# iacopo97/Multimodal-SAM-Adapter

Hardware: AMD Instinct MI355X
Metric: images/sec encoder fwd @1024x1024 RGB+LiDAR ViT-L (higher is better)
Workload: dtype split-operand MFMA: fp16 hi + e5m2 cross terms (h8c / h8 planes, ViT / interaction / up-conv GEMMs) fp16 hi/lo pairs x3 (TwinConvNeXt: f3 planes) and bf16 hi/lo x3 (neck, head); attention blocks with the rel-pos terms fused: every contraction on one fp16 MFMA (q, k, v, P rounded to fp16) in the bloc

## Files before the change

include/mmsa.h:

```cpp
#ifndef MMSA_H
#define MMSA_H
#include <stddef.h>
#include <stdint.h>
#ifdef __cplusplus
extern "C" {
#endif

#ifdef MMSA_BUILDING_LIBRARY
typedef hipStream_t mmsa_stream_t;
#else
typedef void* mmsa_stream_t;
#endif

#include "mmsa_version.h"
int mmsa_version(void);
const char* mmsa_last_error(void);

int mmsa_debug_poison_lds(unsigned pattern, mmsa_stream_t stream);
int mmsa_event_create(void** ev);
int mmsa_event_record(void* ev, mmsa_stream_t stream);
int mmsa_event_elapsed_ms(void* start, void* stop, float* ms);
int mmsa_event_destroy(void* ev);

enum { MMSA_ACT_NONE = 0, MMSA_ACT_GELU = 1, MMSA_ACT_RELU = 2, MMSA_ACT_RELU6 = 3, MMSA_ACT_HSWISH = 4, MMSA_ACT_SIGMOID = 5 };

enum { MMSA_DT_F32 = 0, MMSA_DT_F16 = 1, MMSA_DT_F64 = 2 };

enum { MMSA_FMT_B3 = 0, MMSA_FMT_H8 = 1, MMSA_FMT_H8C = 2, MMSA_FMT_F3 = 3, MMSA_FMT_W8 = 4  };

int mmsa_ms_deform_attn_forward(const void* value, const int64_t* spatial_shapes, const int64_t* level_start_index,
                                const void* sampling_loc, const void* attn_weight, void* out, int batch,
                                int spatial_size, int num_heads, int channels, int num_levels, int num_query,
                                int num_point, int im2col_step, int dtype, mmsa_stream_t stream);

int mmsa_ms_deform_attn_backward(const void* value, const int64_t* spatial_shapes, const int64_t* level_start_index,
                                 const void* sampling_loc, const void* attn_weight, const void* grad_output,
                                 void* grad_value, void* grad_sampling_loc, void* grad_attn_weight, int batch,
                                 int spatial_size, int num_heads, int channels, int num_levels, int num_query,
                                 int num_point, int im2col_step, int dtype, mmsa_stream_t stream);

int mmsa_msda_fused(const float* value, const int64_t* spatial_shapes, const int64_t* level_start_index,
                    const float* raw, long ldraw, const float* ref_points, float* out, long ldo,
                    uint16_t* out_planes, long ldop , int out_fmt , int batch,
                    int spatial_size, int num_heads, int channels, int num_levels, int num_query, int num_point,
                    float* clamp_max , mmsa_stream_t stream);

int mmsa_msda_fused_planes(const uint16_t* value_planes, long ldvp, int lo_bytes, const int64_t* spatial_shapes, const int64_t* level_start_index,
                           const float* raw, long ldraw, const float* ref_points, float* out, long ldo,
                           uint16_t* out_planes, long ldop, int out_fmt, int batch,
                           int spatial_size, int num_heads, int channels, int num_levels, int num_query, int num_point,
                           float* clamp_max, mmsa_stream_t stream);

int mmsa_rowstats_finalize(const float* rowstats, int rows, int strips, int D, float eps, float* mean_rstd, mmsa_stream_t stream);

int mmsa_zero_bytes(void* p, size_t bytes, mmsa_stream_t stream);
int mmsa_gemm_split3(const float* A, const uint16_t* Ap, long lda, long strideA,
                     const uint16_t* Wp, long strideW,
                     const float* bias, long strideBias, const float* colscale, const float* resid, long ldr,
                     long strideR, int resid_mod, float beta, float* C, long ldc, long strideC,
                     uint16_t* Cp, long ldcp, long strideCp, int M, int N, int K,
                     int batch, int act, float alpha, int out_mode, int ps_H, int ps_W, int ps_C, int fmt, int cp_fmt,
                     int max_grid, float* rowstats_out, const float* rownorm_mean_rstd, const float* rownorm_colsum, int flavour,
                     float* clamp_max , mmsa_stream_t stream);

int mmsa_convnext_mlp_fused(const uint16_t* Ap, long lda, long strideA, const uint16_t* W1p, long strideW1, const uint16_t* W2p,
                            long strideW2, const float* b1, const float* b2, const float* gamma, float* x, long ldx, long strideX,
                            int M, int C, int batch, int max_grid, int fmt,
                            float* clamp_max , mmsa_stream_t stream);

int mmsa_split_planes(const float* src, long ld, int rows, int cols, int cols_pad, uint16_t* planes, int kind,
                      float* clamp_max , mmsa_stream_t stream);

int mmsa_attention(const float* qkv, long ldq, const float* qkv_bias, const float* rp, float* out, long ldo, int B,
                   int H, int W, int heads, int head_dim, int window_size, float scale, mmsa_stream_t stream);
int mmsa_attention_planes(const uint16_t* qkv_planes, long ldq, const uint16_t* bias_planes, const float* rp,
                          uint16_t* out_planes, long ldo, int B, int H, int W, int heads, int head_dim,
                          int window_size, float scale, int out_fmt ,
                          int v_fmt ,
                          float* max_abs_logit , mmsa_stream_t stream);

int mmsa_relpos_bias(const float* qkv, long ldq, const float* Rh, const float* Rw, float* rp, int B, int H, int W,
                     int heads, int head_dim, int window_size, mmsa_stream_t stream);
int mmsa_relpos_bias_planes(const uint16_t* qkv_planes, long ldq, const float* Rh, const float* Rw,
                            float* rp, int B, int H, int W, int heads, int head_dim, int window_size, mmsa_stream_t stream);

int mmsa_layernorm_rows(const float* x, long ldx, const float* w, const float* b, float eps, float* y, long ldy,
                        float* y2, long ldy2, uint16_t* y_planes, long ldp ,
                        int rows, int C, int map_mode, int map_H, int map_W, int group_rows, long w_gstride, long y_gcol,
                        int y_wrap, int plane_fmt , float* clamp_max ,
                        mmsa_stream_t stream);

int mmsa_colstats(const float* x, long ldx, long strideB, const float* wrow, int B, int HW, int C, double* out,
                  int out_is_zero , mmsa_stream_t stream);

int mmsa_ffrm_finalize(const double* stats, int B, int HW, int C, float mean_w, float mean_b, const float* Wc,
                       const float* gn_w, const float* gn_b, float* mean_o, float* rstd_o, float* mult_o,
                       float* scratch , mmsa_stream_t stream);
int mmsa_lnhw_apply(const float* x, long ldx, const float* mean, const float* rstd, const float* mult, const float* w,
                    const float* bias, float* y, long ldy, int B, int HW, int C, mmsa_stream_t stream);

int mmsa_dwconv_nhwc(const float* x, long ldx, long xstrideB, const float* w, const float* bias, float* y, long ldy,
                     long ystrideB, uint16_t* y_planes, long ldp, long pstrideB , int planes_fmt ,
                     int B, int H, int W, int C, int k, int act,
                     int imgs_per_group ,
                     float* rowstats ,
                     float* clamp_max , mmsa_stream_t stream);
int mmsa_gconv_nhwc(const float* x, long ldx, const float* w, const float* bias, float* y, long ldy, int B, int H,
                    int W, int G, int cin_g, int cout_g, int k, int act, mmsa_stream_t stream);
int mmsa_gfe_qkv_conv(const float* x, long ldx, const float* w, float* y, long ldy, int B, int H, int W, int G, int cin_g, int cout_g,
                      int* covered, mmsa_stream_t stream);
int mmsa_dwpair_gate(const float* x, long ldx, const float* w, float* y, long ldy, uint16_t* y_planes, long ldp, int B, int H,
                     int W, int C, mmsa_stream_t stream);
int mmsa_im2col_nchw(const float* x, int B, int Ctot, int c0, int Cin, int H, int W, int p, float* out, int Kpad,
                     mmsa_stream_t stream);

long mmsa_gram_tn_scratch_bytes(int B, int P, int c);
int mmsa_gram_tn(const float* X, long ldx, const float* Y, long ldy, long strideB, double* G , int B, int P, int c,
                 int nblk, void* scratch, long scratch_bytes, mmsa_stream_t stream);
int mmsa_chanattn_build(const double* G, const double* sq, long sq_strideB, const double* sk, long sk_strideB,
                        const float* temp, const float* Wp, uint16_t* planes , int B, int c, int cpad,
                        int heads, mmsa_stream_t stream);
int mmsa_gffm_build(const double* E, uint16_t* x_planes, uint16_t* y_planes , int B, int c,
                    int cpad, mmsa_stream_t stream);
int mmsa_gelu_gate(const float* x, long ldx, float* y, long ldy, long rows, int C, mmsa_stream_t stream);
int mmsa_pool_hw(const float* z, long ldz, float* out, long ldo, int B, int H, int W, int C, mmsa_stream_t stream);
int mmsa_ca_apply(const float* z, long ldz, const float* att, long lda, float* out, long ldo,
                  uint16_t* out_planes, long ldp , int B, int H, int W, int C, mmsa_stream_t stream);

int mmsa_tail_fuse(const float* cmap, long ldc, long cstrideB, const float* xtok, long ldx, const float* bn_scale,
                   const float* bn_shift, float* out, uint16_t* out_planes , long ldp,
                   int B, int Hc, int Wc, int Hx, int Wx, int C, mmsa_stream_t stream);

int mmsa_global_attention_planes(const uint16_t* qkv_planes, long ldq, const uint16_t* bias_planes, const uint16_t* relpos_planes,
                                 uint16_t* out_planes, long ldo, int B, int H, int W, int heads, int head_dim, float scale,
                                 int out_fmt , int v_fmt ,
                                 float* max_abs_logit , mmsa_stream_t stream);

int mmsa_window_attention_planes(const uint16_t* qkv_planes, long ldq, const uint16_t* bias_planes,
                                 const uint16_t* relpos_planes, const uint16_t* selector, uint16_t* out_planes, long ldo, int B, int H, int W,
                                 int heads, int head_dim, int window_size, float scale, int out_fmt ,
                                 int v_fmt , float* max_abs_logit , mmsa_stream_t stream);

int mmsa_nchw_to_planes(const float* src, long strideB, uint16_t* planes, long ldp, int B, int C, long HW,
                        mmsa_stream_t stream);
int mmsa_head_fuse(const float* z0, const float* z1, int H1, int W1, const float* z2, int H2, int W2, const float* z3,
                   int H3, int W3, long ld, const float* bn_scale, const float* bn_shift, uint16_t* planes, long ldp,
                   float* out32, long ldo, int B, int H, int W, int C, int act, mmsa_stream_t stream);
int mmsa_tokens_to_nchw(const float* src, long ld, float* dst, int B, long HW, int C, mmsa_stream_t stream);

int mmsa_bilinear_accum_nchw(const float* src, long src_strideB, int B, int C, int hs, int ws, float* dst, int Hd, int Wd, int y0, int x0,
                             int hc, int wc, float* count, int accumulate, mmsa_stream_t stream);
int mmsa_div_count_nchw(float* x, const float* count, int B, int C, long HW, mmsa_stream_t stream);
int mmsa_argmax_nchw(const float* x, unsigned char* out, int B, int C, long HW, mmsa_stream_t stream);
int mmsa_crop_batch_nchw(const float* src, int B, int C, int H, int W, const int* windows, int n, float* dst, int hc, int wc,
                         mmsa_stream_t stream);
int mmsa_slide_argmax(const float* logits, int n, int C, int hs, int ws, const int* windows, unsigned char* out, int B, int H, int W,
                      int hc, int wc, int* uncovered, mmsa_stream_t stream);
int mmsa_slide_argmax_resized(const float* logits, int n, int C, int hs, int ws, const int* windows, unsigned char* out, int B, int H, int W,
                              int hc, int wc, int Hd, int Wd, int Hcut, int Wcut, int* uncovered, mmsa_stream_t stream);

int mmsa_softmax_flip_accum_nchw(const float* logits, float* acc, int B, int C, int H, int W, int flip, int accumulate, int finish_div, mmsa_stream_t stream);
int mmsa_aug_argmax(const float* const* logits, const int* views, int A, int C, const int* windows, const int* windows_host, int total,
                    unsigned char* out, int B, int Ho, int Wo, int* uncovered, mmsa_stream_t stream);

enum { MMSA_PRE_U8 = 0, MMSA_PRE_F32 = 1 };
int mmsa_preprocess_nhwc(const void* src0, int dtype0, const void* src1, int dtype1, int B, int Hs, int Ws, const float* mean,
                         const float* sinv, const int* div255, const int* swap, const float* pad_val, float* dst, int H, int W,
                         mmsa_stream_t stream);
int mmsa_preprocess_crops(const void* src0, int dtype0, const void* src1, int dtype1, int B, int Hs, int Ws, const float* mean,
                          const float* sinv, const int* div255, const int* swap, const float* pad_val, int H, int W, const int* windows,
                          int n, float* dst, int hc, int wc, mmsa_stream_t stream);
int mmsa_preprocess_resize_nhwc(const void* src0, int dtype0, const void* src1, int dtype1, int B, int Hs, int Ws, const float* mean,
                                const float* sinv, const int* div255, const int* swap, const float* pad_val, float* dst, int H, int W,
                                int Hr, int Wr, const int* xofs, const void* xcoef, const int* yofs, const void* ycoef, int fixed_point,
                                mmsa_stream_t stream);
int mmsa_preprocess_resize_crops(const void* src0, int dtype0, const void* src1, int dtype1, int B, int Hs, int Ws, const float* mean,
                                 const float* sinv, const int* div255, const int* swap, const float* pad_val, int H, int W, const int* windows,
                                 int n, float* dst, int hc, int wc, int Hr, int Wr, const int* xofs, const void* xcoef, const int* yofs,
                                 const void* ycoef, int fixed_point, mmsa_stream_t stream);

int mmsa_eval_confusion_u8(const unsigned char* pred, const unsigned char* label, int B, int H, int W, int Hl, int Wl, const unsigned char* lut,
                           int C, const int* ymap, const int* xmap, const int* slots, int n_slots, int64_t* counts, mmsa_stream_t stream);
int mmsa_slide_argmax_eval(const float* logits, int n, int C, int hs, int ws, const int* windows, unsigned char* out, int B, int H, int W,
                           int hc, int wc, int* uncovered, const unsigned char* label, int Hl, int Wl, const unsigned char* lut, const int* ymap,
                           const int* xmap, const int* slots, int n_slots, int64_t* counts, mmsa_stream_t stream);

int mmsa_render_u8(const unsigned char* pred, long pred_image_stride, long pred_row_stride, int B, int h, int w, const unsigned* palette, int npal,
                   int palette_reverse, const unsigned char* src, int Hs, int Ws, int src_reverse, double opacity, double one_minus_opacity,
                   unsigned char* out, mmsa_stream_t stream);
int mmsa_render_denorm_f32(const unsigned char* pred, long pred_image_stride, long pred_row_stride, int B, int h, int w, const unsigned* palette, int npal,
                           int palette_reverse, const float* src, int Cs, int Hs, int Ws, const float* mean, const float* std, int to_rgb, int mul255,
                           double opacity, double one_minus_opacity, unsigned char* out, mmsa_stream_t stream);

#ifdef __cplusplus
}
#endif
#endif
```

include/mmsa_version.h:

```cpp
#ifndef MMSA_VERSION_H
#define MMSA_VERSION_H
#define MMSA_ABI_VERSION 110
#endif
```

multimodal-sam-adapter_amd/csrc/head.hip:

```cpp
#include "common.h"

template <bool VEC>
__global__ __launch_bounds__(256) void nchw_to_planes_kernel(const float* __restrict__ src, long strideB, int C, long HW,
                                                             uint16_t* __restrict__ planes, long ldp) {
  __shared__ float tile[32][257];
  const int b = blockIdx.z;
  const long pix0 = (long)blockIdx.x * 256;
  const int c0 = blockIdx.y * 32;
  const int lane = threadIdx.x & 63, wv = threadIdx.x >> 6;
  const float* sb = src + (long)b * strideB;
  if (VEC) {
    float4 v[8];
#pragma unroll
    for (int j = 0; j < 8; ++j) {
      const int c = c0 + wv * 8 + j;
      const long pix = pix0 + 4 * lane;
      v[j] = (c < C && pix < HW) ? *reinterpret_cast<const float4*>(sb + (long)c * HW + pix) : make_float4(0.f, 0.f, 0.f, 0.f);
    }
#pragma unroll
    for (int j = 0; j < 8; ++j) {
      float* t = &tile[wv * 8 + j][4 * lane];
      t[0] = v[j].x; t[1] = v[j].y; t[2] = v[j].z; t[3] = v[j].w;
    }
  } else {
#pragma unroll
    for (int j = 0; j < 8; ++j) {
      const int cl = wv * 8 + j;
      const int c = c0 + cl;
#pragma unroll
      for (int k = 0; k < 4; ++k) {
        const long pix = pix0 + lane + 64 * k;
        tile[cl][lane + 64 * k] = (c < C && pix < HW) ? sb[(long)c * HW + pix] : 0.f;
      }
    }
  }
  __syncthreads();
  const int q = threadIdx.x & 3;
  const int pl = threadIdx.x >> 2;
#pragma unroll
  for (int k = 0; k < 4; ++k) {
    const int p = pl + 64 * k;
    const long pix = pix0 + p;
    if (pix >= HW) continue;
    float v[8];
#pragma unroll
    for (int j = 0; j < 8; ++j) v[j] = tile[8 * q + j][p];
    uint4 hi, lo;
    split2(v[0], v[1], hi.x, lo.x);
    split2(v[2], v[3], hi.y, lo.y);
    split2(v[4], v[5], hi.z, lo.z);
    split2(v[6], v[7], hi.w, lo.w);
    uint16_t* row = planes + ((long)b * HW + pix) * ldp + (long)blockIdx.y * 64 + 8 * q;
    *reinterpret_cast<uint4*>(row) = hi;
    *reinterpret_cast<uint4*>(row + 32) = lo;
  }
}

extern "C" int mmsa_nchw_to_planes(const float* src, long strideB, uint16_t* planes, long ldp, int B, int C, long HW,
                                   hipStream_t stream) {
  MMSA_CHECK_ARG(src && planes, "nchw_to_planes: null pointer");
  MMSA_CHECK_ARG(B > 0 && C > 0 && HW > 0, "nchw_to_planes: bad shape");
  const int cpad = (C + 31) / 32 * 32;
  MMSA_CHECK_ARG(ldp >= 2L * cpad && ldp % 64 == 0, "nchw_to_planes: planes row stride %ld < 2*%d or not a multiple of 64", ldp, cpad);
  MMSA_CHECK_ARG((reinterpret_cast<uintptr_t>(planes) & 127) == 0, "nchw_to_planes: planes must be 128-byte aligned");
  MMSA_CHECK_ARG(strideB >= (long)C * HW, "nchw_to_planes: image stride %ld < C*HW", strideB);
  dim3 grid(cdiv(HW, 256), cpad / 32, B);
  if ((HW & 3) == 0 && (strideB & 3) == 0 && (reinterpret_cast<uintptr_t>(src) & 15) == 0)
    hipLaunchKernelGGL(nchw_to_planes_kernel<true>, grid, dim3(256), 0, stream, src, strideB, C, HW, planes, ldp);
  else
    hipLaunchKernelGGL(nchw_to_planes_kernel<false>, grid, dim3(256), 0, stream, src, strideB, C, HW, planes, ldp);
  MMSA_CHECK_LAUNCH("nchw_to_planes");
  return MMSA_OK;
}

struct HeadLevels {
  const float* z[3];
  int H[3], W[3];
  float rh[3], rw[3];
};

__global__ __launch_bounds__(256) void head_fuse_kernel(const float* __restrict__ z0, long ld, HeadLevels lv, int nlv,
                                                        const float* __restrict__ bn_scale, const float* __restrict__ bn_shift,
                                                        uint16_t* __restrict__ planes, long ldp, float* __restrict__ out32, long ldo,
                                                        int H, int W, int C, long npix_total, int act) {
  const long pixg = (long)blockIdx.x * 4 + (threadIdx.x >> 6);
  if (pixg >= npix_total) return;
  const int lane = threadIdx.x & 63;
  const unsigned hw = (unsigned)H * (unsigned)W;
  const unsigned pg = (unsigned)pixg;
  const int b = (int)(pg / hw);
  const int rem = (int)(pg - (unsigned)b * hw);
  const int h = rem / W, w = rem - h * W;
  long o00[3], o01[3], o10[3], o11[3];
  float lh[3], lw[3];
#pragma unroll
  for (int i = 0; i < 3; ++i) {
    if (i < nlv) {
      float sh = ((float)h + 0.5f) * lv.rh[i] - 0.5f;
      float sw = ((float)w + 0.5f) * lv.rw[i] - 0.5f;
      sh = sh < 0.f ? 0.f : sh;
      sw = sw < 0.f ? 0.f : sw;
      const int h0 = min((int)sh, lv.H[i] - 1), w0 = min((int)sw, lv.W[i] - 1);
      const int h1 = h0 + (h0 < lv.H[i] - 1 ? 1 : 0), w1 = w0 + (w0 < lv.W[i] - 1 ? 1 : 0);
      lh[i] = sh - (float)h0;
      lw[i] = sw - (float)w0;
      const long base = (long)b * lv.H[i] * lv.W[i];
      o00[i] = (base + (long)h0 * lv.W[i] + w0) * ld;
      o01[i] = (base + (long)h0 * lv.W[i] + w1) * ld;
      o10[i] = (base + (long)h1 * lv.W[i] + w0) * ld;
      o11[i] = (base + (long)h1 * lv.W[i] + w1) * ld;
    } else {
      o00[i] = o01[i] = o10[i] = o11[i] = 0; lh[i] = lw[i] = 0.f;
    }
  }
  for (int c = lane * 8; c < C; c += 512) {
    float v[8];
    float4 t[3][2][4];
    const float4 a = *reinterpret_cast<const float4*>(z0 + pixg * ld + c);
    const float4 d = *reinterpret_cast<const float4*>(z0 + pixg * ld + c + 4);
#pragma unroll
    for (int i = 0; i < 3; ++i) {
      const int il = i < nlv ? i : 0;
      const float* zi = (nlv > 0 ? lv.z[il] : z0 + pixg * ld) + c;
#pragma unroll
      for (int hh = 0; hh < 2; ++hh) {
        t[i][hh][0] = *reinterpret_cast<const float4*>(zi + o00[il] + 4 * hh);
        t[i][hh][1] = *reinterpret_cast<const float4*>(zi + o01[il] + 4 * hh);
        t[i][hh][2] = *reinterpret_cast<const float4*>(zi + o10[il] + 4 * hh);
        t[i][hh][3] = *reinterpret_cast<const float4*>(zi + o11[il] + 4 * hh);
      }
    }
    const float4 s0 = *reinterpret_cast<const float4*>(bn_scale + c), s1 = *reinterpret_cast<const float4*>(bn_scale + c + 4);
    const float4 f0 = *reinterpret_cast<const float4*>(bn_shift + c), f1 = *reinterpret_cast<const float4*>(bn_shift + c + 4);
    __builtin_amdgcn_sched_barrier(0);
    v[0] = a.x; v[1] = a.y; v[2] = a.z; v[3] = a.w; v[4] = d.x; v[5] = d.y; v[6] = d.z; v[7] = d.w;
#pragma unroll
    for (int i = 0; i < 3; ++i) {
      if (i < nlv) {
        const float w00 = (1.f - lh[i]) * (1.f - lw[i]), w01 = (1.f - lh[i]) * lw[i], w10 = lh[i] * (1.f - lw[i]), w11 = lh[i] * lw[i];
#pragma unroll
        for (int hh = 0; hh < 2; ++hh) {
          const float4 t00 = t[i][hh][0], t01 = t[i][hh][1], t10 = t[i][hh][2], t11 = t[i][hh][3];
          v[4 * hh + 0] += w00 * t00.x + w01 * t01.x + w10 * t10.x + w11 * t11.x;
          v[4 * hh + 1] += w00 * t00.y + w01 * t01.y + w10 * t10.y + w11 * t11.y;
          v[4 * hh + 2] += w00 * t00.z + w01 * t01.z + w10 * t10.z + w11 * t11.z;
          v[4 * hh + 3] += w00 * t00.w + w01 * t01.w + w10 * t10.w + w11 * t11.w;
        }
      }
    }
    const float bs[8] = {s0.x, s0.y, s0.z, s0.w, s1.x, s1.y, s1.z, s1.w}, bf[8] = {f0.x, f0.y, f0.z, f0.w, f1.x, f1.y, f1.z, f1.w};
#pragma unroll
    for (int j = 0; j < 8; ++j) v[j] = apply_act(v[j] * bs[j] + bf[j], act);
    if (out32) {
      *reinterpret_cast<float4*>(out32 + pixg * ldo + c) = make_float4(v[0], v[1], v[2], v[3]);
      *reinterpret_cast<float4*>(out32 + pixg * ldo + c + 4) = make_float4(v[4], v[5], v[6], v[7]);
    }
    if (planes) {
      uint4 hi, lo;
      split2(v[0], v[1], hi.x, lo.x);
      split2(v[2], v[3], hi.y, lo.y);
      split2(v[4], v[5], hi.z, lo.z);
      split2(v[6], v[7], hi.w, lo.w);
      uint16_t* row = planes + pixg * ldp + ilv(c);
      *reinterpret_cast<uint4*>(row) = hi;
      *reinterpret_cast<uint4*>(row + 32) = lo;
    }
  }
}

extern "C" int mmsa_head_fuse(const float* z0, const float* z1, int H1, int W1, const float* z2, int H2, int W2, const float* z3,
                              int H3, int W3, long ld, const float* bn_scale, const float* bn_shift, uint16_t* planes, long ldp,
                              float* out32, long ldo, int B, int H, int W, int C, int act, hipStream_t stream) {
  MMSA_CHECK_ARG(z0 && bn_scale && bn_shift && (planes || out32), "head_fuse: null pointer");
  MMSA_CHECK_ARG(((((uintptr_t)bn_scale) | ((uintptr_t)bn_shift) | ((uintptr_t)z0)) & 15) == 0, "head_fuse: z0 / bn_scale / bn_shift must be 16-byte aligned");
  MMSA_CHECK_ARG(B > 0 && H > 0 && W > 0 && C > 0 && C % 8 == 0, "head_fuse: bad shape (C=%d must be a multiple of 8)", C);
  MMSA_CHECK_ARG(ld >= C && ld % 4 == 0, "head_fuse: row stride %ld", ld);
  MMSA_CHECK_ARG(!planes || (ldp >= 2L * ((C + 31) / 32 * 32) && ldp % 64 == 0 && (reinterpret_cast<uintptr_t>(planes) & 127) == 0),
                 "head_fuse: planes stride/alignment");
  MMSA_CHECK_ARG(!out32 || (ldo >= C && ldo % 4 == 0), "head_fuse: fp32 out stride %ld", ldo);
  HeadLevels lv;
  int n = 0;
  const float* zs[3] = {z1, z2, z3};
  const int hs[3] = {H1, H2, H3}, wsz[3] = {W1, W2, W3};
  for (int i = 0; i < 3; ++i) {
    lv.z[i] = nullptr; lv.H[i] = lv.W[i] = 1; lv.rh[i] = lv.rw[i] = 1.f;
  }
  for (int i = 0; i < 3; ++i) {
    if (!zs[i]) continue;
    MMSA_CHECK_ARG(hs[i] > 0 && wsz[i] > 0, "head_fuse: level %d has bad size", i + 1);
    lv.z[n] = zs[i]; lv.H[n] = hs[i]; lv.W[n] = wsz[i];
    lv.rh[n] = (float)hs[i] / (float)H;
    lv.rw[n] = (float)wsz[i] / (float)W;
    ++n;
  }
  const long npix = (long)B * H * W;
  MMSA_CHECK_ARG(npix < (1L << 31), "head_fuse: too many pixels for the 32-bit index arithmetic");
  hipLaunchKernelGGL(head_fuse_kernel, dim3(cdiv(npix, 4)), dim3(256), 0, stream, z0, ld, lv, n, bn_scale, bn_shift, planes, ldp,
                     out32, ldo, H, W, C, npix, act);
  MMSA_CHECK_LAUNCH("head_fuse");
  return MMSA_OK;
}

__global__ __launch_bounds__(256) void tokens_to_nchw_kernel(const float* __restrict__ src, long ld, float* __restrict__ dst, long HW, int C) {
  __shared__ float tile[32][33];
  const int b = blockIdx.z;
  const long pix0 = (long)blockIdx.x * 32;
  const int c0 = blockIdx.y * 32;
  const int tx = threadIdx.x & 31, ty = threadIdx.x >> 5;
#pragma unroll
  for (int k = 0; k < 4; ++k) {
    const int pl = ty + 8 * k;
    const long pix = pix0 + pl;
    const int c = c0 + tx;
    tile[pl][tx] = (pix < HW && c < C) ? src[((long)b * HW + pix) * ld + c] : 0.f;
  }
  __syncthreads();
#pragma unroll
  for (int k = 0; k < 4; ++k) {
    const int c = c0 + ty + 8 * k;
    const long pix = pix0 + tx;
    if (c < C && pix < HW) dst[((long)b * C + c) * HW + pix] = tile[tx][ty + 8 * k];
  }
}

extern "C" int mmsa_tokens_to_nchw(const float* src, long ld, float* dst, int B, long HW, int C, hipStream_t stream) {
  MMSA_CHECK_ARG(src && dst, "tokens_to_nchw: null pointer");
  MMSA_CHECK_ARG(B > 0 && HW > 0 && C > 0 && ld >= C, "tokens_to_nchw: bad shape");
  dim3 grid(cdiv(HW, 32), cdiv(C, 32), B);
  hipLaunchKernelGGL(tokens_to_nchw_kernel, grid, dim3(256), 0, stream, src, ld, dst, HW, C);
  MMSA_CHECK_LAUNCH("tokens_to_nchw");
  return MMSA_OK;
}
```

multimodal-sam-adapter_amd/csrc/tail.hip:

```cpp
#include "common.h"

__global__ __launch_bounds__(256) void tail_fuse_kernel(const float* __restrict__ cmap, long ldc, long cstrideB, const float* __restrict__ xtok, long ldx,
                                                        const float* __restrict__ bn_scale, const float* __restrict__ bn_shift,
                                                        float* __restrict__ out, unsigned short* __restrict__ outp, long ldp,
                                                        int Hc, int Wc, int Hx, int Wx, int C, float rh, float rw) {
  __shared__ float tile[32][33];
  const int b = blockIdx.z;
  const int pix0 = blockIdx.x * 32;
  const int c0 = blockIdx.y * 32;
  const int tx = threadIdx.x & 31, ty = threadIdx.x >> 5;
  const int npix = Hc * Wc;
#pragma unroll
  for (int k = 0; k < 4; ++k) {
    const int pl = ty + 8 * k;
    const int pix = pix0 + pl;
    const int c = c0 + tx;
    float v = 0.f;
    if (pix < npix && c < C) {
      const int h = pix / Wc, w = pix - h * Wc;
      v = cmap[(long)b * cstrideB + (long)pix * ldc + c];
      float sh = ((float)h + 0.5f) * rh - 0.5f;
      float sw = ((float)w + 0.5f) * rw - 0.5f;
      sh = sh < 0.f ? 0.f : sh;
      sw = sw < 0.f ? 0.f : sw;
      const int h0 = (int)sh, w0 = (int)sw;
      const int h1 = h0 + (h0 < Hx - 1 ? 1 : 0), w1 = w0 + (w0 < Wx - 1 ? 1 : 0);
      const float lh = sh - (float)h0, lw = sw - (float)w0;
      if (xtok) {
        const float* xb = xtok + (long)b * Hx * Wx * ldx + c;
        const float v00 = xb[((long)h0 * Wx + w0) * ldx], v01 = xb[((long)h0 * Wx + w1) * ldx];
        const float v10 = xb[((long)h1 * Wx + w0) * ldx], v11 = xb[((long)h1 * Wx + w1) * ldx];
        const float r = (1.f - lh) * ((1.f - lw) * v00 + lw * v01) + lh * ((1.f - lw) * v10 + lw * v11);
        v = v + r;
      }
      v = v * bn_scale[c] + bn_shift[c];
      if (outp) {
        unsigned short hh, ll;
        split_bf16(v, hh, ll);
        unsigned short* q_ = outp + ((long)b * npix + pix) * ldp + ilv(c);
        q_[0] = hh;
        q_[32] = ll;
      }
    }
    tile[pl][tx] = v;
  }
  __syncthreads();
#pragma unroll
  for (int k = 0; k < 4; ++k) {
    const int cl = ty + 8 * k;
    const int c = c0 + cl;
    const int pix = pix0 + tx;
    if (c < C && pix < npix) out[((long)b * C + c) * npix + pix] = tile[tx][cl];
  }
}

__global__ __launch_bounds__(256) void tail_fuse64_kernel(const float* __restrict__ cmap, long ldc, long cstrideB, const float* __restrict__ xtok, long ldx,
                                                          const float* __restrict__ bn_scale, const float* __restrict__ bn_shift,
                                                          float* __restrict__ out, unsigned short* __restrict__ outp, long ldp,
                                                          int Hc, int Wc, int Hx, int Wx, int C, float rh, float rw) {
  __shared__ float tile[64][65];
  const int b = blockIdx.z;
  const int pix0 = blockIdx.x * 64, c0 = blockIdx.y * 64;
  const int t = threadIdx.x;
  const int cg = t & 15, pr = t >> 4;
  const int npix = Hc * Wc;
  const int c = c0 + 4 * cg;
  const bool c_ok = c < C;
  float4 sc = make_float4(0.f, 0.f, 0.f, 0.f), sf = sc;
  if (c_ok) { sc = *reinterpret_cast<const float4*>(bn_scale + c); sf = *reinterpret_cast<const float4*>(bn_shift + c); }
  const float* xb = xtok + (long)b * Hx * Wx * ldx + c;
#pragma unroll
  for (int k = 0; k < 4; ++k) {
    const int pl = pr + 16 * k;
    const int pix = pix0 + pl;
    float4 v = make_float4(0.f, 0.f, 0.f, 0.f);
    const bool ok = pix < npix && c_ok;
    if (ok) {
      const int h = pix / Wc, w = pix - h * Wc;
      v = *reinterpret_cast<const float4*>(cmap + (long)b * cstrideB + (long)pix * ldc + c);
      float sh = ((float)h + 0.5f) * rh - 0.5f;
      float sw = ((float)w + 0.5f) * rw - 0.5f;
      sh = sh < 0.f ? 0.f : sh;
      sw = sw < 0.f ? 0.f : sw;
      const int h0 = (int)sh, w0 = (int)sw;
      const int h1 = h0 + (h0 < Hx - 1 ? 1 : 0), w1 = w0 + (w0 < Wx - 1 ? 1 : 0);
      const float lh = sh - (float)h0, lw = sw - (float)w0;
      if (xtok) {
        const float4 v00 = *reinterpret_cast<const float4*>(xb + ((long)h0 * Wx + w0) * ldx), v01 = *reinterpret_cast<const float4*>(xb + ((long)h0 * Wx + w1) * ldx);
        const float4 v10 = *reinterpret_cast<const float4*>(xb + ((long)h1 * Wx + w0) * ldx), v11 = *reinterpret_cast<const float4*>(xb + ((long)h1 * Wx + w1) * ldx);
#define TF_ONE(f_) { const float r_ = (1.f - lh) * ((1.f - lw) * v00.f_ + lw * v01.f_) + lh * ((1.f - lw) * v10.f_ + lw * v11.f_); v.f_ = (v.f_ + r_) * sc.f_ + sf.f_; }
        TF_ONE(x) TF_ONE(y) TF_ONE(z) TF_ONE(w)
#undef TF_ONE
      } else {
        v.x = v.x * sc.x + sf.x; v.y = v.y * sc.y + sf.y; v.z = v.z * sc.z + sf.z; v.w = v.w * sc.w + sf.w;
      }
    }
    if (outp) {
      unsigned short* row = outp + ((long)b * npix + min(pix, npix - 1)) * ldp;
      store_planes8_pair<1>(row, c & ~7, v, MMSA_FMT_B3, (cg & 1) != 0, ok);
    }
    tile[pl][4 * cg + 0] = v.x; tile[pl][4 * cg + 1] = v.y; tile[pl][4 * cg + 2] = v.z; tile[pl][4 * cg + 3] = v.w;
  }
  __syncthreads();
  const int pg = t & 15, cr = t >> 4;
  const bool vec = (npix & 3) == 0;
#pragma unroll
  for (int k = 0; k < 4; ++k) {
    const int cl = cr + 16 * k;
    const int cc = c0 + cl;
    const int pix = pix0 + 4 * pg;
    if (cc >= C || pix >= npix) continue;
    const float4 o = make_float4(tile[4 * pg][cl], tile[4 * pg + 1][cl], tile[4 * pg + 2][cl], tile[4 * pg + 3][cl]);
    float* dst = out + ((long)b * C + cc) * npix + pix;
    if (vec) *reinterpret_cast<float4*>(dst) = o;
    else {
      dst[0] = o.x;
      if (pix + 1 < npix) dst[1] = o.y;
      if (pix + 2 < npix) dst[2] = o.z;
      if (pix + 3 < npix) dst[3] = o.w;
    }
  }
}

extern "C" int mmsa_tail_fuse(const float* cmap, long ldc, long cstrideB, const float* xtok, long ldx, const float* bn_scale,
                              const float* bn_shift, float* out, unsigned short* out_planes, long ldp, int B, int Hc, int Wc,
                              int Hx, int Wx, int C, hipStream_t stream) {
  MMSA_CHECK_ARG(cmap && bn_scale && bn_shift && out, "tail_fuse: null pointer");
  MMSA_CHECK_ARG(B > 0 && Hc > 0 && Wc > 0 && Hx > 0 && Wx > 0 && C > 0, "tail_fuse: bad shape");
  MMSA_CHECK_ARG(!out_planes || ((C & 31) == 0 && ldp >= 2L * C), "tail_fuse: planes output needs C % 32 == 0 and ldp >= 2C");
  const float rh = (float)Hx / (float)Hc, rw = (float)Wx / (float)Wc;
  const bool old_tiles = MMSA_KNOB("MMSA_TAIL32", 0) != 0;
  const bool wide = !old_tiles && (C & 3) == 0 && (ldc & 3) == 0 && (!xtok || (ldx & 3) == 0) && (cstrideB & 3) == 0 &&
                    ((((uintptr_t)cmap) | ((uintptr_t)xtok) | ((uintptr_t)bn_scale) | ((uintptr_t)bn_shift) | ((uintptr_t)out)) & 15) == 0 &&
                    (!out_planes || ((C & 7) == 0 && (ldp & 7) == 0 && (((uintptr_t)out_planes) & 15) == 0));
  if (wide) {
    dim3 grid64(cdiv((long)Hc * Wc, 64), cdiv(C, 64), B);
    hipLaunchKernelGGL(tail_fuse64_kernel, grid64, dim3(256), 0, stream, cmap, ldc, cstrideB, xtok, ldx, bn_scale, bn_shift, out, out_planes, ldp, Hc, Wc, Hx, Wx, C, rh, rw);
    MMSA_CHECK_LAUNCH("tail_fuse");
    return MMSA_OK;
  }
  dim3 grid(cdiv((long)Hc * Wc, 32), cdiv(C, 32), B);
  hipLaunchKernelGGL(tail_fuse_kernel, grid, dim3(256), 0, stream, cmap, ldc, cstrideB, xtok, ldx, bn_scale, bn_shift, out, out_planes, ldp, Hc, Wc, Hx, Wx, C, rh, rw);
  MMSA_CHECK_LAUNCH("tail_fuse");
  return MMSA_OK;
}
```

multimodal-sam-adapter_amd/mmsa/lib.py:

```python
import ctypes
import os
from ctypes import c_char_p, c_double, c_float, c_int, c_long, c_void_p, POINTER

_HERE = os.path.dirname(os.path.abspath(__file__))
LIB_PATH = os.environ.get("MMSA_LIB") or os.path.join(_HERE, "libmmsa_hip.so")

if not os.path.exists(LIB_PATH):
    raise RuntimeError(
        f"{LIB_PATH} not found: the MI355X HIP library is required (no CPU/PyTorch fallback exists). "
        "Build it with: python multimodal-sam-adapter_amd/build.py")

import torch

_lib = ctypes.CDLL(LIB_PATH)

P = c_void_p
I = c_int
L = c_long
F = c_float

SIGNATURES = {
    "mmsa_version": [],
    "mmsa_last_error": [],
    "mmsa_debug_poison_lds": [ctypes.c_uint, P],
    "mmsa_event_create": [POINTER(c_void_p)],
    "mmsa_event_record": [P, P],
    "mmsa_event_elapsed_ms": [P, P, POINTER(c_float)],
    "mmsa_event_destroy": [P],
    "mmsa_ms_deform_attn_forward": [P, P, P, P, P, P, I, I, I, I, I, I, I, I, I, P],
    "mmsa_ms_deform_attn_backward": [P, P, P, P, P, P, P, P, P, I, I, I, I, I, I, I, I, I, P],
    "mmsa_msda_fused": [P, P, P, P, L, P, P, L, P, L, I, I, I, I, I, I, I, I, P, P],
    "mmsa_msda_fused_planes": [P, L, I, P, P, P, L, P, P, L, P, L, I, I, I, I, I, I, I, I, P, P],
    "mmsa_gemm_split3": [P, P, L, L, P, L, P, L, P, P, L, L, I, F, P, L, L, P, L, L, I, I, I, I, I, F, I, I, I, I, I, I, I, P, P, P, I, P, P],
    "mmsa_convnext_mlp_fused": [P, L, L, P, L, P, L, P, P, P, P, L, L, I, I, I, I, I, P, P],
    "mmsa_rowstats_finalize": [P, I, I, I, F, P, P],
    "mmsa_zero_bytes": [P, ctypes.c_size_t, P],
    "mmsa_split_planes": [P, L, I, I, I, P, I, P, P],
    "mmsa_attention": [P, L, P, P, P, L, I, I, I, I, I, I, F, P],
    "mmsa_attention_planes": [P, L, P, P, P, L, I, I, I, I, I, I, F, I, I, P, P],
    "mmsa_relpos_bias": [P, L, P, P, P, I, I, I, I, I, I, P],
    "mmsa_relpos_bias_planes": [P, L, P, P, P, I, I, I, I, I, I, P],
    "mmsa_layernorm_rows": [P, L, P, P, F, P, L, P, L, P, L, I, I, I, I, I, I, L, L, I, I, P, P],
    "mmsa_colstats": [P, L, L, P, I, I, I, P, I, P],
    "mmsa_ffrm_finalize": [P, I, I, I, F, F, P, P, P, P, P, P, P, P],
    "mmsa_lnhw_apply": [P, L, P, P, P, P, P, P, L, I, I, I, P],
    "mmsa_dwconv_nhwc": [P, L, L, P, P, P, L, L, P, L, L, I, I, I, I, I, I, I, I, P, P, P],
    "mmsa_dwpair_gate": [P, L, P, P, L, P, L, I, I, I, I, P],
    "mmsa_gconv_nhwc": [P, L, P, P, P, L, I, I, I, I, I, I, I, I, P],
    "mmsa_gfe_qkv_conv": [P, L, P, P, L, I, I, I, I, I, I, POINTER(c_int), P],
    "mmsa_im2col_nchw": [P, I, I, I, I, I, I, I, P, I, P],
    "mmsa_gram_tn": [P, L, P, L, L, P, I, I, I, I, P, L, P],
    "mmsa_gram_tn_scratch_bytes": [I, I, I],
    "mmsa_chanattn_build": [P, P, L, P, L, P, P, P, I, I, I, I, P],
    "mmsa_gffm_build": [P, P, P, I, I, I, P],
    "mmsa_gelu_gate": [P, L, P, L, L, I, P],
    "mmsa_pool_hw": [P, L, P, L, I, I, I, I, P],
    "mmsa_ca_apply": [P, L, P, L, P, L, P, L, I, I, I, I, P],
    "mmsa_tail_fuse": [P, L, L, P, L, P, P, P, P, L, I, I, I, I, I, I, P],
    "mmsa_global_attention_planes": [P, L, P, P, P, L, I, I, I, I, I, F, I, I, P, P],
    "mmsa_window_attention_planes": [P, L, P, P, P, P, L, I, I, I, I, I, I, F, I, I, P, P],
    "mmsa_nchw_to_planes": [P, L, P, L, I, I, L, P],
    "mmsa_head_fuse": [P, P, I, I, P, I, I, P, I, I, L, P, P, P, L, P, L, I, I, I, I, I, P],
    "mmsa_tokens_to_nchw": [P, L, P, I, L, I, P],
    "mmsa_bilinear_accum_nchw": [P, L, I, I, I, I, P, I, I, I, I, I, I, P, I, P],
    "mmsa_div_count_nchw": [P, P, I, I, L, P],
    "mmsa_argmax_nchw": [P, P, I, I, L, P],
    "mmsa_crop_batch_nchw": [P, I, I, I, I, P, I, P, I, I, P],
    "mmsa_slide_argmax": [P, I, I, I, I, P, P, I, I, I, I, I, P, P],
    "mmsa_slide_argmax_resized": [P, I, I, I, I, P, P, I, I, I, I, I, I, I, I, I, P, P],
    "mmsa_softmax_flip_accum_nchw": [P, P, I, I, I, I, I, I, I, P],
    "mmsa_aug_argmax": [P, P, I, I, P, P, I, P, I, I, I, P, P],
    "mmsa_preprocess_nhwc": [P, I, P, I, I, I, I, P, P, P, P, P, P, I, I, P],
    "mmsa_preprocess_crops": [P, I, P, I, I, I, I, P, P, P, P, P, I, I, P, I, P, I, I, P],
    "mmsa_preprocess_resize_nhwc": [P, I, P, I, I, I, I, P, P, P, P, P, P, I, I, I, I, P, P, P, P, I, P],
    "mmsa_preprocess_resize_crops": [P, I, P, I, I, I, I, P, P, P, P, P, I, I, P, I, P, I, I, I, I, P, P, P, P, I, P],
    "mmsa_eval_confusion_u8": [P, P, I, I, I, I, I, P, I, P, P, P, I, P, P],
    "mmsa_slide_argmax_eval": [P, I, I, I, I, P, P, I, I, I, I, I, P, P, I, I, P, P, P, P, I, P, P],
    "mmsa_render_u8": [P, L, L, I, I, I, P, I, I, P, I, I, I, c_double, c_double, P, P],
    "mmsa_render_denorm_f32": [P, L, L, I, I, I, P, I, I, P, I, I, I, P, P, I, I, c_double, c_double, P, P],
}
_RESTYPES = {"mmsa_last_error": c_char_p, "mmsa_gram_tn_scratch_bytes": c_long}

for _name, _args in SIGNATURES.items():
    _fn = getattr(_lib, _name)
    _fn.argtypes = _args
    _fn.restype = _RESTYPES.get(_name, c_int)


ABI_VERSION = 110
if _lib.mmsa_version() != ABI_VERSION:
    raise RuntimeError(f"{LIB_PATH}: ABI version {_lib.mmsa_version()} but mmsa/lib.py binds version {ABI_VERSION} (include/mmsa.h MMSA_ABI_VERSION): "
                       "rebuild with python multimodal-sam-adapter_amd/build.py")


def last_error() -> str:
    return _lib.mmsa_last_error().decode()


POISON_LDS = os.environ.get("MMSA_DEBUG_POISON_LDS") == "1"


def call(name, *args):
    if POISON_LDS and not name.startswith(("mmsa_event", "mmsa_debug")) and args:
        _lib.mmsa_debug_poison_lds(0x7FC07FC0, args[-1])
    rc = getattr(_lib, name)(*args)
    if rc != 0:
        raise RuntimeError(f"{name} failed (rc={rc}): {last_error()}")


def version() -> int:
    return _lib.mmsa_version()


raw = _lib
```

Baseline: 65.62.

## Stage bilinear-upsample taps in LDS for head and tail fuse kernels

Adds tiled variants of the head-fuse and tail-fuse kernels. Each block first loads the coarse-level source pixels its output tile needs into shared memory, then does the bilinear interpolation from LDS instead of issuing four global gathers per output pixel. The tiled path is chosen automatically when the levels are coarser than the output and aligned, and the old per-pixel path stays as a fallback. The cost is extra LDS use (up to 80 KB), which may lower occupancy, plus more code paths; the overall effect is small because these are tail kernels in a ViT-L encoder.

```diff
diff --git a/include/mmsa.h b/include/mmsa.h
--- a/include/mmsa.h
+++ b/include/mmsa.h
@@ -130,6 +130,9 @@
 int mmsa_tail_fuse(const float* cmap, long ldc, long cstrideB, const float* xtok, long ldx, const float* bn_scale,
                    const float* bn_shift, float* out, uint16_t* out_planes , long ldp,
                    int B, int Hc, int Wc, int Hx, int Wx, int C, mmsa_stream_t stream);
+int mmsa_tail_fuse_v(const float* cmap, long ldc, long cstrideB, const float* xtok, long ldx, const float* bn_scale,
+                     const float* bn_shift, float* out, uint16_t* out_planes, long ldp,
+                     int B, int Hc, int Wc, int Hx, int Wx, int C, int variant, mmsa_stream_t stream);
 
 int mmsa_global_attention_planes(const uint16_t* qkv_planes, long ldq, const uint16_t* bias_planes, const uint16_t* relpos_planes,
                                  uint16_t* out_planes, long ldo, int B, int H, int W, int heads, int head_dim, float scale,
@@ -146,6 +149,9 @@
 int mmsa_head_fuse(const float* z0, const float* z1, int H1, int W1, const float* z2, int H2, int W2, const float* z3,
                    int H3, int W3, long ld, const float* bn_scale, const float* bn_shift, uint16_t* planes, long ldp,
                    float* out32, long ldo, int B, int H, int W, int C, int act, mmsa_stream_t stream);
+int mmsa_head_fuse_v(const float* z0, const float* z1, int H1, int W1, const float* z2, int H2, int W2, const float* z3,
+                     int H3, int W3, long ld, const float* bn_scale, const float* bn_shift, uint16_t* planes, long ldp,
+                     float* out32, long ldo, int B, int H, int W, int C, int act, int variant, mmsa_stream_t stream);
 int mmsa_tokens_to_nchw(const float* src, long ld, float* dst, int B, long HW, int C, mmsa_stream_t stream);
 
 int mmsa_bilinear_accum_nchw(const float* src, long src_strideB, int B, int C, int hs, int ws, float* dst, int Hd, int Wd, int y0, int x0,
diff --git a/include/mmsa_version.h b/include/mmsa_version.h
--- a/include/mmsa_version.h
+++ b/include/mmsa_version.h
@@ -1,4 +1,4 @@
 #ifndef MMSA_VERSION_H
 #define MMSA_VERSION_H
-#define MMSA_ABI_VERSION 110
+#define MMSA_ABI_VERSION 111
 #endif
diff --git a/multimodal-sam-adapter_amd/csrc/head.hip b/multimodal-sam-adapter_amd/csrc/head.hip
--- a/multimodal-sam-adapter_amd/csrc/head.hip
+++ b/multimodal-sam-adapter_amd/csrc/head.hip
@@ -1,4 +1,5 @@
 #include "common.h"
+#include "resize_taps.h"
 
 template <bool VEC>
 __global__ __launch_bounds__(256) void nchw_to_planes_kernel(const float* __restrict__ src, long strideB, int C, long HW,
@@ -79,6 +80,23 @@
   float rh[3], rw[3];
 };
 
+__device__ __forceinline__ void head_store8(const float* v, long pixg, int c, uint16_t* __restrict__ planes, long ldp, float* __restrict__ out32, long ldo) {
+  if (out32) {
+    *reinterpret_cast<float4*>(out32 + pixg * ldo + c) = make_float4(v[0], v[1], v[2], v[3]);
+    *reinterpret_cast<float4*>(out32 + pixg * ldo + c + 4) = make_float4(v[4], v[5], v[6], v[7]);
+  }
+  if (planes) {
+    uint4 hi, lo;
+    split2(v[0], v[1], hi.x, lo.x);
+    split2(v[2], v[3], hi.y, lo.y);
+    split2(v[4], v[5], hi.z, lo.z);
+    split2(v[6], v[7], hi.w, lo.w);
+    uint16_t* row = planes + pixg * ldp + ilv(c);
+    *reinterpret_cast<uint4*>(row) = hi;
+    *reinterpret_cast<uint4*>(row + 32) = lo;
+  }
+}
+
 __global__ __launch_bounds__(256) void head_fuse_kernel(const float* __restrict__ z0, long ld, HeadLevels lv, int nlv,
                                                         const float* __restrict__ bn_scale, const float* __restrict__ bn_shift,
                                                         uint16_t* __restrict__ planes, long ldp, float* __restrict__ out32, long ldo,
@@ -96,19 +114,14 @@
 #pragma unroll
   for (int i = 0; i < 3; ++i) {
     if (i < nlv) {
-      float sh = ((float)h + 0.5f) * lv.rh[i] - 0.5f;
-      float sw = ((float)w + 0.5f) * lv.rw[i] - 0.5f;
-      sh = sh < 0.f ? 0.f : sh;
-      sw = sw < 0.f ? 0.f : sw;
-      const int h0 = min((int)sh, lv.H[i] - 1), w0 = min((int)sw, lv.W[i] - 1);
-      const int h1 = h0 + (h0 < lv.H[i] - 1 ? 1 : 0), w1 = w0 + (w0 < lv.W[i] - 1 ? 1 : 0);
-      lh[i] = sh - (float)h0;
-      lw[i] = sw - (float)w0;
+      const ResizeTap th = resize_tap(h, lv.rh[i], lv.H[i]), tw = resize_tap(w, lv.rw[i], lv.W[i]);
+      lh[i] = th.l;
+      lw[i] = tw.l;
       const long base = (long)b * lv.H[i] * lv.W[i];
-      o00[i] = (base + (long)h0 * lv.W[i] + w0) * ld;
-      o01[i] = (base + (long)h0 * lv.W[i] + w1) * ld;
-      o10[i] = (base + (long)h1 * lv.W[i] + w0) * ld;
-      o11[i] = (base + (long)h1 * lv.W[i] + w1) * ld;
+      o00[i] = (base + (long)th.i0 * lv.W[i] + tw.i0) * ld;
+      o01[i] = (base + (long)th.i0 * lv.W[i] + tw.i1) * ld;
+      o10[i] = (base + (long)th.i1 * lv.W[i] + tw.i0) * ld;
+      o11[i] = (base + (long)th.i1 * lv.W[i] + tw.i1) * ld;
     } else {
       o00[i] = o01[i] = o10[i] = o11[i] = 0; lh[i] = lw[i] = 0.f;
     }
@@ -137,40 +150,168 @@
 #pragma unroll
     for (int i = 0; i < 3; ++i) {
       if (i < nlv) {
-        const float w00 = (1.f - lh[i]) * (1.f - lw[i]), w01 = (1.f - lh[i]) * lw[i], w10 = lh[i] * (1.f - lw[i]), w11 = lh[i] * lw[i];
-#pragma unroll
-        for (int hh = 0; hh < 2; ++hh) {
-          const float4 t00 = t[i][hh][0], t01 = t[i][hh][1], t10 = t[i][hh][2], t11 = t[i][hh][3];
-          v[4 * hh + 0] += w00 * t00.x + w01 * t01.x + w10 * t10.x + w11 * t11.x;
-          v[4 * hh + 1] += w00 * t00.y + w01 * t01.y + w10 * t10.y + w11 * t11.y;
-          v[4 * hh + 2] += w00 * t00.z + w01 * t01.z + w10 * t10.z + w11 * t11.z;
-          v[4 * hh + 3] += w00 * t00.w + w01 * t01.w + w10 * t10.w + w11 * t11.w;
+        const ResizeWeights wt = resize_weights(lh[i], lw[i]);
+#pragma unroll
+        for (int hh = 0; hh < 2; ++hh) head_tap_add4(v + 4 * hh, wt, t[i][hh][0], t[i][hh][1], t[i][hh][2], t[i][hh][3]);
+      }
+    }
+    const float bs[8] = {s0.x, s0.y, s0.z, s0.w, s1.x, s1.y, s1.z, s1.w}, bf[8] = {f0.x, f0.y, f0.z, f0.w, f1.x, f1.y, f1.z, f1.w};
+#pragma unroll
+    for (int j = 0; j < 8; ++j) v[j] = head_finish(v[j], bs[j], bf[j], act);
+    head_store8(v, pixg, c, planes, ldp, out32, ldo);
+  }
+}
+
+#define HT_CHUNK 128
+#define HT_ROW_F4 32
+#define HT_MAX_LDS (80 * 1024)
+struct HeadBoxes {
+  int bh[3], bw[3];
+  int off[3];
+  int tiles_x, tiles_y;
+};
+
+template <int T>
+__global__ __launch_bounds__(256) void head_fuse_tile_kernel(const float* __restrict__ z0, long ld, HeadLevels lv, int nlv, HeadBoxes bx,
+                                                             const float* __restrict__ bn_scale, const float* __restrict__ bn_shift,
+                                                             uint16_t* __restrict__ planes, long ldp, float* __restrict__ out32, long ldo,
+                                                             int H, int W, int C, int act) {
+  extern __shared__ float4 ht_lds[];
+  const int t = threadIdx.x;
+  const int tx = (int)(blockIdx.x % (unsigned)bx.tiles_x);
+  const int rest = (int)(blockIdx.x / (unsigned)bx.tiles_x);
+  const int ty = rest % bx.tiles_y, b = rest / bx.tiles_y;
+  const int h00 = ty * T, w00 = tx * T;
+  const int c0 = blockIdx.y * HT_CHUNK;
+  const int hl = min(h00 + T - 1, H - 1), wl = min(w00 + T - 1, W - 1);
+
+  int fh[3], fw[3];
+  {
+    const int q = t & 31;
+    const int cq = 8 * (q & 15) + 4 * (q >> 4);
+    const bool c_ok = c0 + cq < C;
+#pragma unroll
+    for (int i = 0; i < 3; ++i) {
+      fh[i] = fw[i] = 0;
+      if (i < nlv) {
+        fh[i] = resize_tap(h00, lv.rh[i], lv.H[i]).i0;
+        fw[i] = resize_tap(w00, lv.rw[i], lv.W[i]).i0;
+        const int nh = min(resize_tap(hl, lv.rh[i], lv.H[i]).i1 - fh[i] + 1, bx.bh[i]);
+        const int nw = min(resize_tap(wl, lv.rw[i], lv.W[i]).i1 - fw[i] + 1, bx.bw[i]);
+        const int nrows = nh * nw;
+        const float rnw = 1.f / (float)nw;
+        const float* zb = lv.z[i] + ((long)b * lv.H[i] * lv.W[i]) * ld + c0 + cq;
+        float4* img = ht_lds + bx.off[i] + q;
+        for (int r0 = t >> 5; r0 < nrows; r0 += 32) {
+          float4 v[4];
+          int at[4];
+#pragma unroll
+          for (int u = 0; u < 4; ++u) {
+            const int r = r0 + 8 * u;
+            v[u] = make_float4(0.f, 0.f, 0.f, 0.f);
+            at[u] = -1;
+            if (r < nrows) {
+              const int rr = (int)(((float)r + 0.5f) * rnw), cc = r - rr * nw;
+              at[u] = (rr * bx.bw[i] + cc) * HT_ROW_F4;
+              if (c_ok) v[u] = *reinterpret_cast<const float4*>(zb + ((long)(fh[i] + rr) * lv.W[i] + fw[i] + cc) * ld);
+            }
+          }
+#pragma unroll
+          for (int u = 0; u < 4; ++u)
+            if (at[u] >= 0) img[at[u]] = v[u];
         }
       }
     }
-    const float bs[8] = {s0.x, s0.y, s0.z, s0.w, s1.x, s1.y, s1.z, s1.w}, bf[8] = {f0.x, f0.y, f0.z, f0.w, f1.x, f1.y, f1.z, f1.w};
-#pragma unroll
-    for (int j = 0; j < 8; ++j) v[j] = apply_act(v[j] * bs[j] + bf[j], act);
-    if (out32) {
-      *reinterpret_cast<float4*>(out32 + pixg * ldo + c) = make_float4(v[0], v[1], v[2], v[3]);
-      *reinterpret_cast<float4*>(out32 + pixg * ldo + c + 4) = make_float4(v[4], v[5], v[6], v[7]);
-    }
-    if (planes) {
-      uint4 hi, lo;
-      split2(v[0], v[1], hi.x, lo.x);
-      split2(v[2], v[3], hi.y, lo.y);
-      split2(v[4], v[5], hi.z, lo.z);
-      split2(v[6], v[7], hi.w, lo.w);
-      uint16_t* row = planes + pixg * ldp + ilv(c);
-      *reinterpret_cast<uint4*>(row) = hi;
-      *reinterpret_cast<uint4*>(row + 32) = lo;
-    }
-  }
-}
-
-extern "C" int mmsa_head_fuse(const float* z0, const float* z1, int H1, int W1, const float* z2, int H2, int W2, const float* z3,
-                              int H3, int W3, long ld, const float* bn_scale, const float* bn_shift, uint16_t* planes, long ldp,
-                              float* out32, long ldo, int B, int H, int W, int C, int act, hipStream_t stream) {
+  }
+  __syncthreads();
+
+  constexpr int RPP = 16 / T;
+  constexpr int NP = T / RPP;
+  const int l16 = t & 15, ps = t >> 4;
+  const int w = w00 + ps % T, hoff = ps / T;
+  const int c = c0 + 8 * l16;
+  const bool wc_ok = w < W && c < C;
+  int iw0[3], iw1[3];
+  float lw[3];
+#pragma unroll
+  for (int i = 0; i < 3; ++i) {
+    iw0[i] = iw1[i] = 0; lw[i] = 0.f;
+    if (i < nlv) {
+      const ResizeTap tw = resize_tap(min(w, W - 1), lv.rw[i], lv.W[i]);
+      iw0[i] = min(max(tw.i0 - fw[i], 0), bx.bw[i] - 1);
+      iw1[i] = min(max(tw.i1 - fw[i], 0), bx.bw[i] - 1);
+      lw[i] = tw.l;
+    }
+  }
+  float4 s0 = make_float4(0.f, 0.f, 0.f, 0.f), s1 = s0, f0 = s0, f1 = s0;
+  if (c < C) {
+    s0 = *reinterpret_cast<const float4*>(bn_scale + c); s1 = *reinterpret_cast<const float4*>(bn_scale + c + 4);
+    f0 = *reinterpret_cast<const float4*>(bn_shift + c); f1 = *reinterpret_cast<const float4*>(bn_shift + c + 4);
+  }
+  const float bs[8] = {s0.x, s0.y, s0.z, s0.w, s1.x, s1.y, s1.z, s1.w}, bf[8] = {f0.x, f0.y, f0.z, f0.w, f1.x, f1.y, f1.z, f1.w};
+  for (int p0 = 0; p0 < NP; p0 += 4) {
+    float4 a[4], d[4];
+#pragma unroll
+    for (int g = 0; g < 4; ++g) {
+      const int h = h00 + (p0 + g) * RPP + hoff;
+      a[g] = d[g] = make_float4(0.f, 0.f, 0.f, 0.f);
+      if (wc_ok && h < H) {
+        const long pixg = ((long)b * H + h) * W + w;
+        a[g] = *reinterpret_cast<const float4*>(z0 + pixg * ld + c);
+        d[g] = *reinterpret_cast<const float4*>(z0 + pixg * ld + c + 4);
+      }
+    }
+    __builtin_amdgcn_sched_barrier(0);
+#pragma unroll
+    for (int g = 0; g < 4; ++g) {
+      const int h = h00 + (p0 + g) * RPP + hoff;
+      if (!(wc_ok && h < H)) continue;
+      const long pixg = ((long)b * H + h) * W + w;
+      float v[8] = {a[g].x, a[g].y, a[g].z, a[g].w, d[g].x, d[g].y, d[g].z, d[g].w};
+#pragma unroll
+      for (int i = 0; i < 3; ++i) {
+        if (i < nlv) {
+          const ResizeTap th = resize_tap(h, lv.rh[i], lv.H[i]);
+          const int ih0 = min(max(th.i0 - fh[i], 0), bx.bh[i] - 1), ih1 = min(max(th.i1 - fh[i], 0), bx.bh[i] - 1);
+          const float4* img = ht_lds + bx.off[i] + l16;
+          const float4* r00 = img + (ih0 * bx.bw[i] + iw0[i]) * HT_ROW_F4;
+          const float4* r01 = img + (ih0 * bx.bw[i] + iw1[i]) * HT_ROW_F4;
+          const float4* r10 = img + (ih1 * bx.bw[i] + iw0[i]) * HT_ROW_F4;
+          const float4* r11 = img + (ih1 * bx.bw[i] + iw1[i]) * HT_ROW_F4;
+          const ResizeWeights wt = resize_weights(th.l, lw[i]);
+#pragma unroll
+          for (int hh = 0; hh < 2; ++hh) head_tap_add4(v + 4 * hh, wt, r00[16 * hh], r01[16 * hh], r10[16 * hh], r11[16 * hh]);
+        }
+      }
+#pragma unroll
+      for (int j = 0; j < 8; ++j) v[j] = head_finish(v[j], bs[j], bf[j], act);
+      head_store8(v, pixg, c, planes, ldp, out32, ldo);
+    }
+  }
+}
+
+static int head_tile_plan(const HeadLevels& lv, int n, int H, int W, HeadBoxes& bx) {
+  for (int T = 16; T >= 8; T >>= 1) {
+    int rows = 0;
+    for (int i = 0; i < 3; ++i) {
+      bx.bh[i] = bx.bw[i] = 1; bx.off[i] = 0;
+      if (i >= n) continue;
+      bx.bh[i] = resize_tap_box_max(T, lv.rh[i], lv.H[i]);
+      bx.bw[i] = resize_tap_box_max(T, lv.rw[i], lv.W[i]);
+      bx.off[i] = rows * HT_ROW_F4;
+      rows += bx.bh[i] * bx.bw[i];
+    }
+    if ((long)rows * HT_ROW_F4 * 16 <= HT_MAX_LDS) {
+      bx.tiles_x = cdiv(W, T); bx.tiles_y = cdiv(H, T);
+      return T;
+    }
+  }
+  return 0;
+}
+
+extern "C" int mmsa_head_fuse_v(const float* z0, const float* z1, int H1, int W1, const float* z2, int H2, int W2, const float* z3,
+                                int H3, int W3, long ld, const float* bn_scale, const float* bn_shift, uint16_t* planes, long ldp,
+                                float* out32, long ldo, int B, int H, int W, int C, int act, int variant, hipStream_t stream) {
   MMSA_CHECK_ARG(z0 && bn_scale && bn_shift && (planes || out32), "head_fuse: null pointer");
   MMSA_CHECK_ARG(((((uintptr_t)bn_scale) | ((uintptr_t)bn_shift) | ((uintptr_t)z0)) & 15) == 0, "head_fuse: z0 / bn_scale / bn_shift must be 16-byte aligned");
   MMSA_CHECK_ARG(B > 0 && H > 0 && W > 0 && C > 0 && C % 8 == 0, "head_fuse: bad shape (C=%d must be a multiple of 8)", C);
@@ -178,6 +319,7 @@
   MMSA_CHECK_ARG(!planes || (ldp >= 2L * ((C + 31) / 32 * 32) && ldp % 64 == 0 && (reinterpret_cast<uintptr_t>(planes) & 127) == 0),
                  "head_fuse: planes stride/alignment");
   MMSA_CHECK_ARG(!out32 || (ldo >= C && ldo % 4 == 0), "head_fuse: fp32 out stride %ld", ldo);
+  MMSA_CHECK_ARG(variant >= 0 && variant <= 2, "head_fuse: variant %d (0 = automatic, 1 = per pixel, 2 = tiled)", variant);
   HeadLevels lv;
   int n = 0;
   const float* zs[3] = {z1, z2, z3};
@@ -185,20 +327,52 @@
   for (int i = 0; i < 3; ++i) {
     lv.z[i] = nullptr; lv.H[i] = lv.W[i] = 1; lv.rh[i] = lv.rw[i] = 1.f;
   }
+  bool coarse = true, aligned = true;
   for (int i = 0; i < 3; ++i) {
     if (!zs[i]) continue;
     MMSA_CHECK_ARG(hs[i] > 0 && wsz[i] > 0, "head_fuse: level %d has bad size", i + 1);
     lv.z[n] = zs[i]; lv.H[n] = hs[i]; lv.W[n] = wsz[i];
     lv.rh[n] = (float)hs[i] / (float)H;
     lv.rw[n] = (float)wsz[i] / (float)W;
+    coarse = coarse && hs[i] <= H && wsz[i] <= W;
+    aligned = aligned && (((uintptr_t)zs[i]) & 15) == 0;
     ++n;
   }
   const long npix = (long)B * H * W;
   MMSA_CHECK_ARG(npix < (1L << 31), "head_fuse: too many pixels for the 32-bit index arithmetic");
+  HeadBoxes bx;
+  const int T = (n > 0 && coarse && aligned) ? head_tile_plan(lv, n, H, W, bx) : 0;
+  const long ntiles = T ? (long)B * bx.tiles_x * bx.tiles_y : 0;
+  const bool tiled_ok = T != 0 && ntiles < (1L << 31) && cdiv(C, HT_CHUNK) <= 65535;
+  MMSA_CHECK_ARG(variant != 2 || tiled_ok, "head_fuse: variant 2 (tiled) needs at least one level, none finer than the output, 16-byte aligned levels "
+                 "and tap boxes within %d bytes of LDS", HT_MAX_LDS);
+  if (tiled_ok && variant != 1) {
+    static MmsaPerDevice per_dev_ = {};
+    (void)mmsa_per_device(per_dev_, [] {
+      (void)hipFuncSetAttribute((const void*)head_fuse_tile_kernel<16>, hipFuncAttributeMaxDynamicSharedMemorySize, HT_MAX_LDS);
+      (void)hipFuncSetAttribute((const void*)head_fuse_tile_kernel<8>, hipFuncAttributeMaxDynamicSharedMemorySize, HT_MAX_LDS);
+    });
+    int rows = 0;
+    for (int i = 0; i < n; ++i) rows += bx.bh[i] * bx.bw[i];
+    const size_t lds = (size_t)rows * HT_ROW_F4 * 16;
+    const dim3 grid((unsigned)ntiles, cdiv(C, HT_CHUNK));
+    if (T == 16)
+      hipLaunchKernelGGL(head_fuse_tile_kernel<16>, grid, dim3(256), lds, stream, z0, ld, lv, n, bx, bn_scale, bn_shift, planes, ldp, out32, ldo, H, W, C, act);
+    else
+      hipLaunchKernelGGL(head_fuse_tile_kernel<8>, grid, dim3(256), lds, stream, z0, ld, lv, n, bx, bn_scale, bn_shift, planes, ldp, out32, ldo, H, W, C, act);
+    MMSA_CHECK_LAUNCH("head_fuse");
+    return MMSA_OK;
+  }
   hipLaunchKernelGGL(head_fuse_kernel, dim3(cdiv(npix, 4)), dim3(256), 0, stream, z0, ld, lv, n, bn_scale, bn_shift, planes, ldp,
                      out32, ldo, H, W, C, npix, act);
   MMSA_CHECK_LAUNCH("head_fuse");
   return MMSA_OK;
+}
+
+extern "C" int mmsa_head_fuse(const float* z0, const float* z1, int H1, int W1, const float* z2, int H2, int W2, const float* z3,
+                              int H3, int W3, long ld, const float* bn_scale, const float* bn_shift, uint16_t* planes, long ldp,
+                              float* out32, long ldo, int B, int H, int W, int C, int act, hipStream_t stream) {
+  return mmsa_head_fuse_v(z0, z1, H1, W1, z2, H2, W2, z3, H3, W3, ld, bn_scale, bn_shift, planes, ldp, out32, ldo, B, H, W, C, act, 0, stream);
 }
 
 __global__ __launch_bounds__(256) void tokens_to_nchw_kernel(const float* __restrict__ src, long ld, float* __restrict__ dst, long HW, int C) {
diff --git a/multimodal-sam-adapter_amd/csrc/resize_taps.h b/multimodal-sam-adapter_amd/csrc/resize_taps.h
--- /dev/null
+++ b/multimodal-sam-adapter_amd/csrc/resize_taps.h
@@ -0,0 +1,65 @@
+#pragma once
+#include <math.h>
+
+#if defined(__HIPCC__)
+#define RT_HD __host__ __device__ __forceinline__
+#else
+#define RT_HD static inline
+#endif
+
+struct ResizeTap {
+  int i0, i1;
+  float l;
+};
+
+RT_HD ResizeTap resize_tap(int d, float r, int n) {
+  float s = fmaf((float)d + 0.5f, r, -0.5f);
+  s = s < 0.f ? 0.f : s;
+  const int f = (int)s;
+  ResizeTap t;
+  t.i0 = f < n - 1 ? f : n - 1;
+  t.i1 = t.i0 + (t.i0 < n - 1 ? 1 : 0);
+  t.l = s - (float)t.i0;
+  return t;
+}
+
+struct ResizeBox { int first, count; };
+RT_HD ResizeBox resize_tap_box(int d0, int T, int nd, float r, int n) {
+  const int dl = d0 + T - 1 < nd - 1 ? d0 + T - 1 : nd - 1;
+  ResizeBox b;
+  b.first = resize_tap(d0, r, n).i0;
+  b.count = resize_tap(dl, r, n).i1 - b.first + 1;
+  return b;
+}
+
+RT_HD int resize_tap_box_max(int T, float r, int n) {
+  const int e = (int)floor((double)(T - 1) * (double)r + 1e-4) + 3;
+  return e < n ? e : n;
+}
+
+#if defined(__HIPCC__)
+struct ResizeWeights { float w00, w01, w10, w11; };
+__device__ __forceinline__ ResizeWeights resize_weights(float lh, float lw) {
+  ResizeWeights w;
+  w.w00 = (1.f - lh) * (1.f - lw); w.w01 = (1.f - lh) * lw; w.w10 = lh * (1.f - lw); w.w11 = lh * lw;
+  return w;
+}
+__device__ __forceinline__ void head_tap_add(float& v, const ResizeWeights w, float t00, float t01, float t10, float t11) {
+  v += fmaf(w.w11, t11, fmaf(w.w10, t10, fmaf(w.w00, t00, w.w01 * t01)));
+}
+__device__ __forceinline__ void head_tap_add4(float* v, const ResizeWeights w, const float4 t00, const float4 t01, const float4 t10, const float4 t11) {
+  head_tap_add(v[0], w, t00.x, t01.x, t10.x, t11.x);
+  head_tap_add(v[1], w, t00.y, t01.y, t10.y, t11.y);
+  head_tap_add(v[2], w, t00.z, t01.z, t10.z, t11.z);
+  head_tap_add(v[3], w, t00.w, t01.w, t10.w, t11.w);
+}
+__device__ __forceinline__ float head_finish(float v, float bn_scale, float bn_shift, int act) { return apply_act(fmaf(v, bn_scale, bn_shift), act); }
+
+template <bool LOWER_FROM_V11>
+__device__ __forceinline__ float tail_one(float c, float v00, float v01, float v10, float v11, float lh, float lw, float bn_scale, float bn_shift) {
+  const float a = fmaf(lw, v01, (1.f - lw) * v00);
+  const float b = LOWER_FROM_V11 ? fmaf(lw, v11, (1.f - lw) * v10) : fmaf(1.f - lw, v10, lw * v11);
+  const float r = fmaf(1.f - lh, a, lh * b);
+  return fmaf(c + r, bn_scale, bn_shift);
+}
+#endif
diff --git a/multimodal-sam-adapter_amd/csrc/tail.hip b/multimodal-sam-adapter_amd/csrc/tail.hip
--- a/multimodal-sam-adapter_amd/csrc/tail.hip
+++ b/multimodal-sam-adapter_amd/csrc/tail.hip
@@ -1,4 +1,5 @@
 #include "common.h"
+#include "resize_taps.h"
 
 __global__ __launch_bounds__(256) void tail_fuse_kernel(const float* __restrict__ cmap, long ldc, long cstrideB, const float* __restrict__ xtok, long ldx,
                                                         const float* __restrict__ bn_scale, const float* __restrict__ bn_shift,
@@ -19,21 +20,15 @@
     if (pix < npix && c < C) {
       const int h = pix / Wc, w = pix - h * Wc;
       v = cmap[(long)b * cstrideB + (long)pix * ldc + c];
-      float sh = ((float)h + 0.5f) * rh - 0.5f;
-      float sw = ((float)w + 0.5f) * rw - 0.5f;
-      sh = sh < 0.f ? 0.f : sh;
-      sw = sw < 0.f ? 0.f : sw;
-      const int h0 = (int)sh, w0 = (int)sw;
-      const int h1 = h0 + (h0 < Hx - 1 ? 1 : 0), w1 = w0 + (w0 < Wx - 1 ? 1 : 0);
-      const float lh = sh - (float)h0, lw = sw - (float)w0;
+      const ResizeTap th = resize_tap(h, rh, Hx), tw = resize_tap(w, rw, Wx);
       if (xtok) {
         const float* xb = xtok + (long)b * Hx * Wx * ldx + c;
-        const float v00 = xb[((long)h0 * Wx + w0) * ldx], v01 = xb[((long)h0 * Wx + w1) * ldx];
-        const float v10 = xb[((long)h1 * Wx + w0) * ldx], v11 = xb[((long)h1 * Wx + w1) * ldx];
-        const float r = (1.f - lh) * ((1.f - lw) * v00 + lw * v01) + lh * ((1.f - lw) * v10 + lw * v11);
-        v = v + r;
-      }
-      v = v * bn_scale[c] + bn_shift[c];
+        const float v00 = xb[((long)th.i0 * Wx + tw.i0) * ldx], v01 = xb[((long)th.i0 * Wx + tw.i1) * ldx];
+        const float v10 = xb[((long)th.i1 * Wx + tw.i0) * ldx], v11 = xb[((long)th.i1 * Wx + tw.i1) * ldx];
+        v = tail_one<true>(v, v00, v01, v10, v11, th.l, tw.l, bn_scale[c], bn_shift[c]);
+      } else {
+        v = v * bn_scale[c] + bn_shift[c];
+      }
       if (outp) {
         unsigned short hh, ll;
         split_bf16(v, hh, ll);
@@ -54,11 +49,12 @@
   }
 }
 
-__global__ __launch_bounds__(256) void tail_fuse64_kernel(const float* __restrict__ cmap, long ldc, long cstrideB, const float* __restrict__ xtok, long ldx,
-                                                          const float* __restrict__ bn_scale, const float* __restrict__ bn_shift,
-                                                          float* __restrict__ out, unsigned short* __restrict__ outp, long ldp,
-                                                          int Hc, int Wc, int Hx, int Wx, int C, float rh, float rw) {
-  __shared__ float tile[64][65];
+#define TT_MAX_BW 34
+template <bool STAGED>
+__device__ __forceinline__ void tail_fuse64_body(float (*tile)[65], float4* taps, int bw, const float* __restrict__ cmap, long ldc, long cstrideB,
+                                                 const float* __restrict__ xtok, long ldx, const float* __restrict__ bn_scale, const float* __restrict__ bn_shift,
+                                                 float* __restrict__ out, unsigned short* __restrict__ outp, long ldp,
+                                                 int Hc, int Wc, int Hx, int Wx, int C, float rh, float rw) {
   const int b = blockIdx.z;
   const int pix0 = blockIdx.x * 64, c0 = blockIdx.y * 64;
   const int t = threadIdx.x;
@@ -69,6 +65,43 @@
   float4 sc = make_float4(0.f, 0.f, 0.f, 0.f), sf = sc;
   if (c_ok) { sc = *reinterpret_cast<const float4*>(bn_scale + c); sf = *reinterpret_cast<const float4*>(bn_shift + c); }
   const float* xb = xtok + (long)b * Hx * Wx * ldx + c;
+  float4 vc[4];
+  int fw = 0;
+  if (STAGED) {
+    const int hrow = pix0 / Wc, w0 = pix0 - hrow * Wc;
+    const ResizeTap th = resize_tap(hrow, rh, Hx);
+    fw = resize_tap(w0, rw, Wx).i0;
+    const int nw = min(resize_tap(min(w0 + 63, Wc - 1), rw, Wx).i1 - fw + 1, bw);
+    const int nitems = 2 * nw * 16;
+    const float* xs = xtok + (long)b * Hx * Wx * ldx + c0;
+    float4 sv[5];
+#pragma unroll
+    for (int u = 0; u < 5; ++u) {
+      const int it = t + 256 * u;
+      sv[u] = make_float4(0.f, 0.f, 0.f, 0.f);
+      if (it < nitems) {
+        const int j = it & 15, pos = it >> 4;
+        const int row = pos >= nw ? 1 : 0, col = pos - row * nw;
+        if (c0 + 4 * j < C) sv[u] = *reinterpret_cast<const float4*>(xs + ((long)(row ? th.i1 : th.i0) * Wx + fw + col) * ldx + 4 * j);
+      }
+    }
+#pragma unroll
+    for (int k = 0; k < 4; ++k) {
+      const int pix = pix0 + pr + 16 * k;
+      vc[k] = make_float4(0.f, 0.f, 0.f, 0.f);
+      if (pix < npix && c_ok) vc[k] = *reinterpret_cast<const float4*>(cmap + (long)b * cstrideB + (long)pix * ldc + c);
+    }
+#pragma unroll
+    for (int u = 0; u < 5; ++u) {
+      const int it = t + 256 * u;
+      if (it < nitems) {
+        const int j = it & 15, pos = it >> 4;
+        const int row = pos >= nw ? 1 : 0, col = pos - row * nw;
+        taps[(row * bw + col) * 16 + j] = sv[u];
+      }
+    }
+    __syncthreads();
+  }
 #pragma unroll
   for (int k = 0; k < 4; ++k) {
     const int pl = pr + 16 * k;
@@ -77,18 +110,18 @@
     const bool ok = pix < npix && c_ok;
     if (ok) {
       const int h = pix / Wc, w = pix - h * Wc;
-      v = *reinterpret_cast<const float4*>(cmap + (long)b * cstrideB + (long)pix * ldc + c);
-      float sh = ((float)h + 0.5f) * rh - 0.5f;
-      float sw = ((float)w + 0.5f) * rw - 0.5f;
-      sh = sh < 0.f ? 0.f : sh;
-      sw = sw < 0.f ? 0.f : sw;
-      const int h0 = (int)sh, w0 = (int)sw;
-      const int h1 = h0 + (h0 < Hx - 1 ? 1 : 0), w1 = w0 + (w0 < Wx - 1 ? 1 : 0);
-      const float lh = sh - (float)h0, lw = sw - (float)w0;
-      if (xtok) {
-        const float4 v00 = *reinterpret_cast<const float4*>(xb + ((long)h0 * Wx + w0) * ldx), v01 = *reinterpret_cast<const float4*>(xb + ((long)h0 * Wx + w1) * ldx);
-        const float4 v10 = *reinterpret_cast<const float4*>(xb + ((long)h1 * Wx + w0) * ldx), v11 = *reinterpret_cast<const float4*>(xb + ((long)h1 * Wx + w1) * ldx);
-#define TF_ONE(f_) { const float r_ = (1.f - lh) * ((1.f - lw) * v00.f_ + lw * v01.f_) + lh * ((1.f - lw) * v10.f_ + lw * v11.f_); v.f_ = (v.f_ + r_) * sc.f_ + sf.f_; }
+      v = STAGED ? vc[k] : *reinterpret_cast<const float4*>(cmap + (long)b * cstrideB + (long)pix * ldc + c);
+      const ResizeTap th = resize_tap(h, rh, Hx), tw = resize_tap(w, rw, Wx);
+      if (STAGED) {
+        const int i0 = min(max(tw.i0 - fw, 0), bw - 1), i1 = min(max(tw.i1 - fw, 0), bw - 1);
+        const float4 v00 = taps[i0 * 16 + cg], v01 = taps[i1 * 16 + cg], v10 = taps[(bw + i0) * 16 + cg], v11 = taps[(bw + i1) * 16 + cg];
+#define TF_ONE(f_) v.f_ = tail_one<false>(v.f_, v00.f_, v01.f_, v10.f_, v11.f_, th.l, tw.l, sc.f_, sf.f_);
+        TF_ONE(x) TF_ONE(y) TF_ONE(z) TF_ONE(w)
+#undef TF_ONE
+      } else if (xtok) {
+        const float4 v00 = *reinterpret_cast<const float4*>(xb + ((long)th.i0 * Wx + tw.i0) * ldx), v01 = *reinterpret_cast<const float4*>(xb + ((long)th.i0 * Wx + tw.i1) * ldx);
+        const float4 v10 = *reinterpret_cast<const float4*>(xb + ((long)th.i1 * Wx + tw.i0) * ldx), v11 = *reinterpret_cast<const float4*>(xb + ((long)th.i1 * Wx + tw.i1) * ldx);
+#define TF_ONE(f_) v.f_ = tail_one<false>(v.f_, v00.f_, v01.f_, v10.f_, v11.f_, th.l, tw.l, sc.f_, sf.f_);
         TF_ONE(x) TF_ONE(y) TF_ONE(z) TF_ONE(w)
 #undef TF_ONE
       } else {
@@ -122,9 +155,26 @@
   }
 }
 
-extern "C" int mmsa_tail_fuse(const float* cmap, long ldc, long cstrideB, const float* xtok, long ldx, const float* bn_scale,
+__global__ __launch_bounds__(256) void tail_fuse64_kernel(const float* __restrict__ cmap, long ldc, long cstrideB, const float* __restrict__ xtok, long ldx,
+                                                          const float* __restrict__ bn_scale, const float* __restrict__ bn_shift,
+                                                          float* __restrict__ out, unsigned short* __restrict__ outp, long ldp,
+                                                          int Hc, int Wc, int Hx, int Wx, int C, float rh, float rw) {
+  __shared__ float tile[64][65];
+  tail_fuse64_body<false>(tile, nullptr, 0, cmap, ldc, cstrideB, xtok, ldx, bn_scale, bn_shift, out, outp, ldp, Hc, Wc, Hx, Wx, C, rh, rw);
+}
+
+__global__ __launch_bounds__(256) void tail_fuse64_tile_kernel(const float* __restrict__ cmap, long ldc, long cstrideB, const float* __restrict__ xtok, long ldx,
+                                                               const float* __restrict__ bn_scale, const float* __restrict__ bn_shift,
+                                                               float* __restrict__ out, unsigned short* __restrict__ outp, long ldp,
+                                                               int Hc, int Wc, int Hx, int Wx, int C, float rh, float rw, int bw) {
+  __shared__ float tile[64][65];
+  extern __shared__ float4 tt_taps[];
+  tail_fuse64_body<true>(tile, tt_taps, bw, cmap, ldc, cstrideB, xtok, ldx, bn_scale, bn_shift, out, outp, ldp, Hc, Wc, Hx, Wx, C, rh, rw);
+}
+
+extern "C" int mmsa_tail_fuse_v(const float* cmap, long ldc, long cstrideB, const float* xtok, long ldx, const float* bn_scale,
                               const float* bn_shift, float* out, unsigned short* out_planes, long ldp, int B, int Hc, int Wc,
-                              int Hx, int Wx, int C, hipStream_t stream) {
+                              int Hx, int Wx, int C, int variant, hipStream_t stream) {
   MMSA_CHECK_ARG(cmap && bn_scale && bn_shift && out, "tail_fuse: null pointer");
   MMSA_CHECK_ARG(B > 0 && Hc > 0 && Wc > 0 && Hx > 0 && Wx > 0 && C > 0, "tail_fuse: bad shape");
   MMSA_CHECK_ARG(!out_planes || ((C & 31) == 0 && ldp >= 2L * C), "tail_fuse: planes output needs C % 32 == 0 and ldp >= 2C");
@@ -133,6 +183,16 @@
   const bool wide = !old_tiles && (C & 3) == 0 && (ldc & 3) == 0 && (!xtok || (ldx & 3) == 0) && (cstrideB & 3) == 0 &&
                     ((((uintptr_t)cmap) | ((uintptr_t)xtok) | ((uintptr_t)bn_scale) | ((uintptr_t)bn_shift) | ((uintptr_t)out)) & 15) == 0 &&
                     (!out_planes || ((C & 7) == 0 && (ldp & 7) == 0 && (((uintptr_t)out_planes) & 15) == 0));
+  MMSA_CHECK_ARG(variant >= 0 && variant <= 2, "tail_fuse: variant %d (0 = automatic, 1 = direct loads, 2 = tiled)", variant);
+  const int bw = resize_tap_box_max(64, rw, Wx);
+  const bool tiled_ok = wide && xtok && Wc % 64 == 0 && 2 * Wx <= Wc && bw <= TT_MAX_BW;
+  MMSA_CHECK_ARG(variant != 2 || tiled_ok, "tail_fuse: variant 2 (tiled) needs xtok, Wc %% 64 == 0, Wx <= Wc / 2 and the 16-byte aligned operands of the 64 x 64 kernel");
+  if (tiled_ok && variant != 1) {
+    dim3 grid64(cdiv((long)Hc * Wc, 64), cdiv(C, 64), B);
+    hipLaunchKernelGGL(tail_fuse64_tile_kernel, grid64, dim3(256), (size_t)2 * bw * 16 * sizeof(float4), stream, cmap, ldc, cstrideB, xtok, ldx, bn_scale, bn_shift, out, out_planes, ldp, Hc, Wc, Hx, Wx, C, rh, rw, bw);
+    MMSA_CHECK_LAUNCH("tail_fuse");
+    return MMSA_OK;
+  }
   if (wide) {
     dim3 grid64(cdiv((long)Hc * Wc, 64), cdiv(C, 64), B);
     hipLaunchKernelGGL(tail_fuse64_kernel, grid64, dim3(256), 0, stream, cmap, ldc, cstrideB, xtok, ldx, bn_scale, bn_shift, out, out_planes, ldp, Hc, Wc, Hx, Wx, C, rh, rw);
@@ -144,3 +204,9 @@
   MMSA_CHECK_LAUNCH("tail_fuse");
   return MMSA_OK;
 }
+
+extern "C" int mmsa_tail_fuse(const float* cmap, long ldc, long cstrideB, const float* xtok, long ldx, const float* bn_scale,
+                              const float* bn_shift, float* out, unsigned short* out_planes, long ldp, int B, int Hc, int Wc,
+                              int Hx, int Wx, int C, hipStream_t stream) {
+  return mmsa_tail_fuse_v(cmap, ldc, cstrideB, xtok, ldx, bn_scale, bn_shift, out, out_planes, ldp, B, Hc, Wc, Hx, Wx, C, 0, stream);
+}
diff --git a/multimodal-sam-adapter_amd/mmsa/lib.py b/multimodal-sam-adapter_amd/mmsa/lib.py
--- a/multimodal-sam-adapter_amd/mmsa/lib.py
+++ b/multimodal-sam-adapter_amd/mmsa/lib.py
@@ -57,10 +57,12 @@
     "mmsa_pool_hw": [P, L, P, L, I, I, I, I, P],
     "mmsa_ca_apply": [P, L, P, L, P, L, P, L, I, I, I, I, P],
     "mmsa_tail_fuse": [P, L, L, P, L, P, P, P, P, L, I, I, I, I, I, I, P],
+    "mmsa_tail_fuse_v": [P, L, L, P, L, P, P, P, P, L, I, I, I, I, I, I, I, P],
     "mmsa_global_attention_planes": [P, L, P, P, P, L, I, I, I, I, I, F, I, I, P, P],
     "mmsa_window_attention_planes": [P, L, P, P, P, P, L, I, I, I, I, I, I, F, I, I, P, P],
     "mmsa_nchw_to_planes": [P, L, P, L, I, I, L, P],
     "mmsa_head_fuse": [P, P, I, I, P, I, I, P, I, I, L, P, P, P, L, P, L, I, I, I, I, I, P],
+    "mmsa_head_fuse_v": [P, P, I, I, P, I, I, P, I, I, L, P, P, P, L, P, L, I, I, I, I, I, I, P],
     "mmsa_tokens_to_nchw": [P, L, P, I, L, I, P],
     "mmsa_bilinear_accum_nchw": [P, L, I, I, I, I, P, I, I, I, I, I, I, P, I, P],
     "mmsa_div_count_nchw": [P, P, I, I, L, P],
@@ -87,7 +89,7 @@
     _fn.restype = _RESTYPES.get(_name, c_int)
 
 
-ABI_VERSION = 110
+ABI_VERSION = 111
 if _lib.mmsa_version() != ABI_VERSION:
     raise RuntimeError(f"{LIB_PATH}: ABI version {_lib.mmsa_version()} but mmsa/lib.py binds version {ABI_VERSION} (include/mmsa.h MMSA_ABI_VERSION): "
                        "rebuild with python multimodal-sam-adapter_amd/build.py")
```

Result: no change. 66.00, median of 6 (+0.6%).
